# HyHuang1995/sp_orb_slam

Hardware: AMD Instinct MI355X
Metric: frames/sec SuperPoint extract (752x480, 1k kpts) (higher is better)
Workload: dtype f32

## Files before the change

sp_orb_slam_amd/csrc/conv_f32.hip:

```cpp
#include <type_traits>
#include <utility>

#include "spfe_kernels.h"
#include "../../include/spfe_exact_math.h"

namespace spfe {

typedef float f32x16 __attribute__((ext_vector_type(16)));

template <int KS, int TH>
struct Geo {
  static constexpr int HALO = KS / 2;
  static constexpr int ROWS = TH + 2 * HALO;
  static constexpr int COLS = 32 + 2 * HALO;
  static constexpr int ROWP = (KS == 3) ? 36 : 32;
  static constexpr int PLANE_RAW = ROWS * ROWP;
  static constexpr int PLANE = PLANE_RAW + ((2 - PLANE_RAW % 8) + 8) % 8;
};

typedef int i32x4 __attribute__((ext_vector_type(4)));
#define SPFE_OOB 0x80000000u

template <int NITER, int NWITER>
struct Pipe {
  float4 va[NITER];
  float4 vw[NWITER];
  int dst[NITER];
  unsigned voff[NITER];
  unsigned woff[NWITER];
  __amdgpu_buffer_rsrc_t rin, rw;
  const float *at[8];
  const float *bBase;
  float *nA, *nW;
};

template <int NR, int NT>
struct EpiCtx {
  __amdgpu_buffer_rsrc_t rout;
  unsigned rbase[NR][NT];
  float bias[NT];
  int xlim;
  unsigned pixstep;
};

__device__ __forceinline__ float max4_finite(float a, float b, float c, float d) {
  float m;
  asm("v_max3_f32 %0, %1, %2, %3\n\tv_max_f32 %0, %0, %4" : "=&v"(m) : "v"(a), "v"(b), "v"(c), "v"(d));
  return m;
}

template <int MT, int NT, bool POOL, bool RELU, int E>
__device__ __forceinline__ void epi_store(const EpiCtx<POOL ? MT / 2 : MT, NT> &e, const f32x16 (&acc)[MT][NT]) {
  constexpr int NEPI_ = POOL ? (MT / 2) * NT * 8 : MT * NT * 16;
  if constexpr (E >= NEPI_) {
    return;
  } else if constexpr (!POOL) {
    constexpr int j = E / (MT * 16), i = (E / 16) % MT, r = E % 16;
    constexpr int xr = (r & 3) + 8 * (r >> 2);
    float v = acc[i][j][r] + e.bias[j];
    if (RELU) v = v > 0.0f ? v : 0.0f;
    const unsigned off = xr < e.xlim ? e.rbase[i][j] : SPFE_OOB;
    __builtin_amdgcn_raw_buffer_store_b32(__float_as_int(v), e.rout, off, xr * e.pixstep, 0);
  } else {
    constexpr int ip = E / (NT * 8), j = (E / 8) % NT, r = 2 * (E % 8), i0 = 2 * ip;
    constexpr int xr = (r & 3) + 8 * (r >> 2);
    const float m = max4_finite(acc[i0][j][r], acc[i0][j][r + 1], acc[i0 + 1][j][r], acc[i0 + 1][j][r + 1]);
    float v = m + e.bias[j];
    if (RELU) v = v > 0.0f ? v : 0.0f;
    const unsigned off = xr < e.xlim ? e.rbase[ip][j] : SPFE_OOB;
    __builtin_amdgcn_raw_buffer_store_b32(__float_as_int(v), e.rout, off, (xr >> 1) * e.pixstep, 0);
  }
}

constexpr int F1_PROWS = 12, F1_PCOLS = 36, F1_PATCH = F1_PROWS * F1_PCOLS;

template <int NITER>
struct Fuse1a {
  float4 w[9], bias;
  float px[9];
  float4 o;
  unsigned pb[NITER];
  const float *patch;
  float *patch_next;
  const float *wsrc;
  const float *bsrc;
  __amdgpu_buffer_rsrc_t rimg;
  unsigned poff[2];
  unsigned pidx[2];
  unsigned pval[2];
  bool fill;
};
struct NoFuse {};

constexpr int F1_SUBS = 10;
template <int NITER, int IT, int SUB, int PLANE, int NWITER>
__device__ __forceinline__ void fuse_piece(Fuse1a<NITER> &z, Pipe<NITER, NWITER> &c) {
  if constexpr (SUB == 0) {
    const unsigned b = z.pb[IT] == ~0u ? 0u : z.pb[IT];
#pragma unroll
    for (int t = 0; t < 9; ++t) z.px[t] = z.patch[b + (t / 3) * F1_PCOLS + t % 3];
  } else if constexpr (SUB <= 8) {
    constexpr int j = (SUB - 1) / 2, half = (SUB - 1) % 2;
    float acc = half == 0 ? 0.0f : (j == 0 ? z.o.x : (j == 1 ? z.o.y : (j == 2 ? z.o.z : z.o.w)));
#pragma unroll
    for (int t = half * 5; t < (half == 0 ? 5 : 9); ++t) {
      const float wt = j == 0 ? z.w[t].x : (j == 1 ? z.w[t].y : (j == 2 ? z.w[t].z : z.w[t].w));
      acc = __builtin_fmaf(z.px[t], wt, acc);
    }
    if constexpr (half == 1) {
      const float bj = j == 0 ? z.bias.x : (j == 1 ? z.bias.y : (j == 2 ? z.bias.z : z.bias.w));
      acc = acc + bj;
      acc = acc > 0.0f ? acc : 0.0f;
      if (c.voff[IT] == SPFE_OOB) acc = 0.0f;
    }
    if constexpr (j == 0) z.o.x = acc;
    else if constexpr (j == 1) z.o.y = acc;
    else if constexpr (j == 2) z.o.z = acc;
    else z.o.w = acc;
  } else {
    float *d = c.nA + c.dst[IT];
    d[0] = z.o.x;
    d[PLANE] = z.o.y;
    d[2 * PLANE] = z.o.z;
    d[3 * PLANE] = z.o.w;
  }
}

template <int STEP, int NSTEP, bool FIRST, int KC, int KS, int MT, int NT, int PLANE, int ROWP, int NITER,
          int NWITER, bool POOL, bool RELU, bool FUSE, class FZ>
__device__ __forceinline__ void k_steps(float (&a)[2][MT], float (&bb)[2][NT], f32x16 (&acc)[MT][NT],
                                        const f32x16 (&accPrev)[MT][NT], Pipe<NITER, NWITER> &c,
                                        const EpiCtx<POOL ? MT / 2 : MT, NT> &e, FZ &fz) {
  if constexpr (STEP < NSTEP) {
    constexpr int NLDA = FUSE ? 0 : NITER;
    constexpr int NLD = NLDA + NWITER;
    constexpr int L0 = 1, W0 = NSTEP - NLD - 1;
    constexpr int NEPI = POOL ? (MT / 2) * NT * 8 : MT * NT * 16;
    constexpr int EPS = (NEPI + (NSTEP - 3)) / (NSTEP - 2);
    constexpr int cur = STEP & 1, nxt = cur ^ 1;
    static_assert(L0 + NLD <= W0, "loads and LDS writes of a stage must not overlap");
    constexpr int M = MT * NT;
    if constexpr (STEP >= 1) __builtin_amdgcn_s_waitcnt(0xC07F);
#pragma unroll
    for (int m = 0; m < M; ++m) {
      if (m == 0) {
        if constexpr (STEP + 1 < NSTEP) {
          constexpr int tap = (STEP + 1) / (KC / 2), t = (STEP + 1) % (KC / 2);
          constexpr int dy = tap / KS, dx = tap % KS;
#pragma unroll
          for (int i = 0; i < MT; ++i) {
            if constexpr (KC / 2 <= 8) a[nxt][i] = c.at[t][(i + dy) * ROWP + dx];
            else a[nxt][i] = c.at[0][(2 * t) * PLANE + (i + dy) * ROWP + dx];
          }
#pragma unroll
          for (int j = 0; j < NT; ++j) bb[nxt][j] = c.bBase[j * (KS * KS * KC * 32) + (tap * KC + 2 * t) * 32];
        }
      }
      if (m == 1 % M) {
        if constexpr (STEP >= L0 && STEP - L0 < NLD) {
          constexpr int it = STEP - L0;
          if constexpr (it < NLDA) {
            const i32x4 v = __builtin_amdgcn_raw_buffer_load_b128(c.rin, c.voff[it], 0, 0);
            c.va[it] = make_float4(__int_as_float(v.x), __int_as_float(v.y), __int_as_float(v.z), __int_as_float(v.w));
          } else {
            constexpr int wi = it - NLDA;
            const i32x4 v = __builtin_amdgcn_raw_buffer_load_b128(c.rw, c.woff[wi], 0, 0);
            c.vw[wi] = make_float4(__int_as_float(v.x), __int_as_float(v.y), __int_as_float(v.z), __int_as_float(v.w));
          }
        }
      }
      if (m == 2 % M) {
        if constexpr (FIRST && STEP >= 1) {
          constexpr int e0 = (STEP - 1) * EPS;
          [&]<int... Qs>(std::integer_sequence<int, Qs...>) {
            (epi_store<MT, NT, POOL, RELU, e0 + Qs>(e, accPrev), ...);
          }(std::make_integer_sequence<int, EPS>{});
        }
      }
      if (m == 3 % M) {
        if constexpr (STEP >= W0 && STEP - W0 < NLD) {
          constexpr int it = STEP - W0;
          if constexpr (it < NLDA) {
            float *d = c.nA + c.dst[it];
            d[0] = c.va[it].x;
            d[PLANE] = c.va[it].y;
            d[2 * PLANE] = c.va[it].z;
            d[3 * PLANE] = c.va[it].w;
          } else {
            constexpr int wi = it - NLDA;
            *reinterpret_cast<float4 *>(reinterpret_cast<char *>(c.nW) + c.woff[wi]) = c.vw[wi];
          }
        }
      }
      if (m == 1 % M) {
        if constexpr (FUSE) {
          constexpr int F0 = 12;
          static_assert(L0 + NLD <= F0 && F0 + F1_SUBS * NITER <= NSTEP, "fused conv1a schedule does not fit the stage");
          if constexpr (STEP >= F0 && STEP < F0 + F1_SUBS * NITER)
            fuse_piece<NITER, (STEP - F0) / F1_SUBS, (STEP - F0) % F1_SUBS, PLANE, NWITER>(fz, c);
        }
      }
      if (m == 3 % M) {
        if constexpr (FUSE) {
          static_assert(58 < W0, "fused conv1a schedule does not fit the stage");
          if constexpr (STEP >= 2 && STEP < 11) fz.w[STEP - 2] = *reinterpret_cast<const float4 *>(fz.wsrc + (STEP - 2) * 64);
          if constexpr (STEP == 11) fz.bias = *reinterpret_cast<const float4 *>(fz.bsrc);
          if constexpr (STEP == 50) {
            if (fz.fill) {
              fz.pval[0] = __builtin_amdgcn_raw_buffer_load_b8(fz.rimg, fz.poff[0], 0, 0);
              fz.pval[1] = __builtin_amdgcn_raw_buffer_load_b8(fz.rimg, fz.poff[1], 0, 0);
            }
          }
          if constexpr (STEP == 58) {
            if (fz.fill) {
              if (fz.pidx[0] < F1_PATCH) fz.patch_next[fz.pidx[0]] = spfe_pixel_to_float((uint8_t)fz.pval[0]);
              if (fz.pidx[1] < F1_PATCH) fz.patch_next[fz.pidx[1]] = spfe_pixel_to_float((uint8_t)fz.pval[1]);
            }
          }
        }
      }
      __builtin_amdgcn_sched_barrier(0);
      {
        const int i = m / NT, j = m % NT;
        if constexpr (FIRST && STEP == 0) {
          f32x16 z;
#pragma unroll
          for (int r = 0; r < 16; ++r) z[r] = 0.0f;
          acc[i][j] = __builtin_amdgcn_mfma_f32_32x32x2f32(a[cur][i], bb[cur][j], z, 0, 0, 0);
        } else {
          acc[i][j] = __builtin_amdgcn_mfma_f32_32x32x2f32(a[cur][i], bb[cur][j], acc[i][j], 0, 0, 0);
        }
      }
      __builtin_amdgcn_sched_barrier(0);
    }
    k_steps<STEP + 1, NSTEP, FIRST, KC, KS, MT, NT, PLANE, ROWP, NITER, NWITER, POOL, RELU, FUSE, FZ>(a, bb, acc, accPrev, c, e, fz);
  }
}

template <int LAYER, int CIN, int KS, int KC, int WM, int WN, int MT, int NT, bool POOL, bool RELU>
// ... 91 lines not shown
    c.rw = __builtin_amdgcn_make_buffer_rsrc(const_cast<float *>(wb), 0, valid ? (unsigned)SLAB_BYTES : 0u, 0x00020000);
  };

  aim_tile(i_tx, i_ty);
  aim_stage(i_nb, i_b, 0, true);
  FZ fz;
  [[maybe_unused]] float *sP = smem + 2 * BUF;
  [[maybe_unused]] int pcur = 0;
  [[maybe_unused]] int php[2] = {0, 0}, pwp[2] = {0, 0};
  if constexpr (FUSE) {
    const int qq = tid % Q;
#pragma unroll
    for (int it = 0; it < NITER; ++it) {
      const int i = tid + it * 256, pix = i / Q;
      fz.pb[it] = i < NITEM ? (unsigned)((pix / G::COLS) * F1_PCOLS + pix % G::COLS) : ~0u;
    }
#pragma unroll
    for (int k = 0; k < 2; ++k) {
      const int i = tid + k * 256;
      fz.pidx[k] = i < F1_PATCH ? (unsigned)i : 0xffffu;
      php[k] = i / F1_PCOLS;
      pwp[k] = i % F1_PCOLS;
      fz.poff[k] = SPFE_OOB;
      fz.pval[k] = 0u;
    }
    fz.fill = false;
    fz.patch = sP;
    fz.patch_next = sP + F1_PATCH;
    fz.rimg = __builtin_amdgcn_make_buffer_rsrc(const_cast<uint8_t *>(p.img), 0, 0u, 0x00020000);
    fz.wsrc = p.w1a + qq * 4;
    fz.bsrc = p.b1a + qq * 4;
    {
      const uint8_t *ib = p.img + (size_t)i_b * H * W;
#pragma unroll
      for (int k = 0; k < 2; ++k) {
        const int gy = i_ty * TH - 2 + php[k], gx = i_tx * 32 - 2 + pwp[k];
        const bool in = (unsigned)gy < (unsigned)H && (unsigned)gx < (unsigned)W;
        if (fz.pidx[k] < F1_PATCH) sP[fz.pidx[k]] = in ? spfe_pixel_to_float(ib[(size_t)gy * W + gx]) : 0.0f;
      }
    }
    __syncthreads();
#pragma unroll
    for (int t = 0; t < 9; ++t) fz.w[t] = *reinterpret_cast<const float4 *>(fz.wsrc + t * 64);
    fz.bias = *reinterpret_cast<const float4 *>(fz.bsrc);
    c.nA = smem;
    [&]<int... I>(std::integer_sequence<int, I...>) {
      (fuse_piece<NITER, I / F1_SUBS, I % F1_SUBS, PLANE, NWITER>(fz, c), ...);
    }(std::make_integer_sequence<int, F1_SUBS * NITER>{});
  } else {
#pragma unroll
    for (int it = 0; it < NITER; ++it) {
      const i32x4 v = __builtin_amdgcn_raw_buffer_load_b128(c.rin, c.voff[it], 0, 0);
      c.va[it] = make_float4(__int_as_float(v.x), __int_as_float(v.y), __int_as_float(v.z), __int_as_float(v.w));
    }
  }
#pragma unroll
  for (int it = 0; it < NWITER; ++it) {
    const i32x4 v = __builtin_amdgcn_raw_buffer_load_b128(c.rw, c.woff[it], 0, 0);
    c.vw[it] = make_float4(__int_as_float(v.x), __int_as_float(v.y), __int_as_float(v.z), __int_as_float(v.w));
  }
  if constexpr (!FUSE) {
#pragma unroll
    for (int it = 0; it < NITER; ++it) {
      float *d = smem + c.dst[it];
      d[0] = c.va[it].x;
      d[PLANE] = c.va[it].y;
      d[2 * PLANE] = c.va[it].z;
      d[3 * PLANE] = c.va[it].w;
    }
  }
#pragma unroll
  for (int it = 0; it < NWITER; ++it)
    *reinterpret_cast<float4 *>(reinterpret_cast<char *>(smem + KC * PLANE) + c.woff[it]) = c.vw[it];
  __syncthreads();

  f32x16 accA[MT][NT], accB[MT][NT];
#pragma unroll
  for (int i = 0; i < MT; ++i)
#pragma unroll
    for (int j = 0; j < NT; ++j)
#pragma unroll
      for (int r = 0; r < 16; ++r) { accA[i][j][r] = 0.0f; accB[i][j][r] = 0.0f; }

  constexpr int NR = POOL ? MT / 2 : MT;
  using Epi = EpiCtx<NR, NT>;
  Epi epi;
  epi.rout = __builtin_amdgcn_make_buffer_rsrc(p.out, 0, 0u, 0x00020000);
#pragma unroll
  for (int j = 0; j < NT; ++j) {
    epi.bias[j] = 0.0f;
#pragma unroll
    for (int q = 0; q < NR; ++q) epi.rbase[q][j] = SPFE_OOB;
  }
  epi.xlim = 0; epi.pixstep = out_pix_bytes;
  bool more = true;

  auto aim_epi = [&](Epi &e, int nb, int tx, int ty, int b) {
    float *obase = p.out + (size_t)b * Ho * Wo * p.out_stride + p.out_choff;
    e.rout = __builtin_amdgcn_make_buffer_rsrc(obase, 0, frame_out_bytes, 0x00020000);
    const int y0 = ty * TH + wm * MT, x0 = tx * 32 + 4 * hi;
    e.xlim = W - x0;
    e.pixstep = out_pix_bytes;
    const int ylim = H - y0;
    const unsigned rowstep = (unsigned)Wo * out_pix_bytes;
#pragma unroll
    for (int j = 0; j < NT; ++j) {
      const int co = nb * 64 + (wn * NT + j) * 32 + l31;
      const unsigned pix = POOL ? (unsigned)((y0 >> 1) * Wo + (x0 >> 1)) : (unsigned)(y0 * W + x0);
      const unsigned obase = pix * out_pix_bytes + (unsigned)co * 4u;
#pragma unroll
      for (int q = 0; q < NR; ++q)
        e.rbase[q][j] = (co < p.cout_real && (POOL ? 2 * q : q) < ylim) ? obase + q * rowstep : SPFE_OOB;
      e.bias[j] = p.bias[co];
    }
  };

  Epi epi_next;
  auto run_tile = [&](f32x16(&acc)[MT][NT], const f32x16(&accPrev)[MT][NT]) {
    int n_nb = i_nb + d_nb, n_tx = i_tx + d_tx, n_ty = i_ty + d_ty, n_b = i_b + d_b;
    if (n_nb >= p.nblk) { n_nb -= p.nblk; ++n_tx; }
    if (n_tx >= p.tiles_x) { n_tx -= p.tiles_x; ++n_ty; }
    if (n_ty >= p.tiles_y) { n_ty -= p.tiles_y; ++n_b; }
    const bool have_next_item = w + gper < hi_w;
    aim_epi(epi_next, i_nb, i_tx, i_ty, i_b);
    auto stage = [&]<bool FIRST>(std::bool_constant<FIRST>, const int chunk) {
      const bool last = chunk == NCHUNK - 1;
      if (!last) {
        aim_stage(i_nb, i_b, chunk + 1, true);
      } else {
        aim_tile(n_tx, n_ty);
        aim_stage(n_nb, n_b, 0, have_next_item);
      }
      if constexpr (FUSE) {
        const int produced = last ? 0 : chunk + 1;
        const int qq = tid % Q;
        fz.wsrc = p.w1a + produced * KC + qq * 4;
        fz.bsrc = p.b1a + produced * KC + qq * 4;
        fz.patch = sP + (last ? pcur ^ 1 : pcur) * F1_PATCH;
        fz.patch_next = sP + (pcur ^ 1) * F1_PATCH;
        fz.fill = chunk == NCHUNK - 2 && have_next_item;
        if (fz.fill) {
          fz.rimg = __builtin_amdgcn_make_buffer_rsrc(const_cast<uint8_t *>(p.img) + (size_t)n_b * H * W, 0,
                                                      (unsigned)(H * W), 0x00020000);
#pragma unroll
          for (int k = 0; k < 2; ++k) {
            const int gy = n_ty * TH - 2 + php[k], gx = n_tx * 32 - 2 + pwp[k];
            fz.poff[k] = ((unsigned)gy < (unsigned)H && (unsigned)gx < (unsigned)W) ? (unsigned)(gy * W + gx) : SPFE_OOB;
          }
        }
      }
      const int buf = chunk & 1;
      float *cA = smem + buf * BUF;
      c.nA = smem + (buf ^ 1) * BUF;
      c.nW = c.nA + KC * PLANE;
#pragma unroll
      for (int t = 0; t < (KC / 2 <= 8 ? KC / 2 : 1); ++t)
        c.at[t] = cA + (2 * t + hi) * PLANE + (wm * MT) * ROWP + l31;
      c.bBase = cA + KC * PLANE + (wn * NT) * (TAPS * KC * 32) + hi * 32 + l31;
      float a[2][MT], bb[2][NT];
#pragma unroll
      for (int i = 0; i < MT; ++i) a[0][i] = c.at[0][i * ROWP];
#pragma unroll
      for (int j = 0; j < NT; ++j) bb[0][j] = c.bBase[j * (TAPS * KC * 32)];
      k_steps<0, NSTEP, FIRST, KC, KS, MT, NT, PLANE, ROWP, NITER, NWITER, POOL, RELU, FUSE, FZ>(a, bb, acc, accPrev, c, epi, fz);
      __syncthreads();
    };
    static_assert(NCHUNK >= 2 && NCHUNK % 2 == 0, "the stage that carries the epilogue is not the tile's last; buf = chunk & 1");
    stage(std::true_type{}, 0);
#pragma unroll 1
    for (int chunk = 1; chunk < NCHUNK; ++chunk) stage(std::false_type{}, chunk);
    epi = epi_next;
    if constexpr (FUSE) pcur ^= 1;
    more = have_next_item;
    w += gper;
    i_nb = n_nb; i_tx = n_tx; i_ty = n_ty; i_b = n_b;
  };

  bool lastA = true;
  while (true) {
    run_tile(accA, accB);
    lastA = true;
    if (!more) break;
    run_tile(accB, accA);
    lastA = false;
    if (!more) break;
  }
  {
    constexpr int NEPI = POOL ? (MT / 2) * NT * 8 : MT * NT * 16;
    auto flush = [&](const f32x16(&acc)[MT][NT]) {
      [&]<int... E>(std::integer_sequence<int, E...>) {
        (epi_store<MT, NT, POOL, RELU, E>(epi, acc), ...);
      }(std::make_integer_sequence<int, NEPI>{});
    };
    if (lastA) flush(accA); else flush(accB);
  }
}

template <int LAYER, int CIN, int KS, int KC, int WM, int WN, int MT, int NT, bool POOL, bool RELU>
static hipError_t launch_one(const ConvParams &p, hipStream_t s) {
  constexpr int TH = WM * MT;
  using G = Geo<KS, TH>;
  constexpr size_t lds = (2 * (size_t)(KC * G::PLANE + KS * KS * KC * 64) + (LAYER == 2 ? 2 * F1_PATCH : 0)) * sizeof(float);
  static_assert(lds <= 160 * 1024, "double buffer must fit the 160 KB LDS");
  auto k = conv_f32_kernel<LAYER, CIN, KS, KC, WM, WN, MT, NT, POOL, RELU>;
  static LdsLimitOnce lds_once;
  if (hipError_t e = raise_lds_limit(lds_once, reinterpret_cast<const void *>(k), (int)lds); e != hipSuccess) return e;
  const int total = p.nblk * p.tiles_x * p.tiles_y * p.B;
  int grid = p.num_cus > 0 ? p.num_cus : 256;
  grid &= ~7;
  if (grid < 8) grid = 8;
  (void)total;
  hipLaunchKernelGGL(k, dim3(grid), dim3(64 * WM * WN), lds, s, p);
  return hipGetLastError();
}

int conv_kc(int ksize) { return ksize == 3 ? 16 : 64; }
int conv_tile_rows(int tile_mode) { return tile_mode == 1 ? 4 : (tile_mode == 2 || tile_mode == 4 ? 16 : (tile_mode == 3 ? 2 : 8)); }

hipError_t launch_conv_f32(const ConvParams &p, int cin, int ksize, bool pool, bool relu,
                           int tile_mode, int layer_tag, hipStream_t s) {
  const bool small_tile = tile_mode == 1;
  if (tile_mode == 3 && ksize == 3 && relu && !pool) {
    if (cin == 64) return launch_one<0, 64, 3, 16, 2, 2, 1, 1, false, true>(p, s);
    if (cin == 128) return launch_one<0, 128, 3, 16, 2, 2, 1, 1, false, true>(p, s);
    return hipErrorInvalidValue;
  }
  if (tile_mode == 4 && ksize == 3 && relu && pool && cin == 64 && layer_tag == 1)
    return launch_one<1, 64, 3, 16, 4, 1, 4, 2, true, true>(p, s);
  if (tile_mode == 2 && ksize == 3 && relu) {
    if (layer_tag == 1 && cin == 64 && pool) return launch_one<1, 64, 3, 16, 8, 1, 2, 2, true, true>(p, s);
    if (cin == 64 && pool) return launch_one<0, 64, 3, 16, 8, 1, 2, 2, true, true>(p, s);
    if (cin == 64 && !pool) return launch_one<0, 64, 3, 16, 8, 1, 2, 2, false, true>(p, s);
    if (cin == 128 && pool) return launch_one<0, 128, 3, 16, 8, 1, 2, 2, true, true>(p, s);
    if (cin == 128 && !pool) return launch_one<0, 128, 3, 16, 8, 1, 2, 2, false, true>(p, s);
    return hipErrorInvalidValue;
  }
  if (layer_tag == 1 && cin == 64 && ksize == 3 && pool && relu && !small_tile)
    return launch_one<1, 64, 3, 16, 4, 1, 2, 2, true, true>(p, s);
  if (layer_tag == 2 && cin == 64 && ksize == 3 && pool && relu && !small_tile && p.img && p.w1a && p.b1a)
    return launch_one<2, 64, 3, 16, 4, 1, 2, 2, true, true>(p, s);
#define SPFE_CONV(CIN_, KS_, KC_, WM_, WN_, MT_, NT_, POOL_, RELU_)                       \
  if (cin == CIN_ && ksize == KS_ && pool == POOL_ && relu == RELU_ &&                    \
      small_tile == (WM_ * MT_ == 4))                                                     \
    return launch_one<0, CIN_, KS_, KC_, WM_, WN_, MT_, NT_, POOL_, RELU_>(p, s);
  SPFE_CONV(64, 3, 16, 4, 1, 2, 2, true, true)
  SPFE_CONV(64, 3, 16, 4, 1, 2, 2, false, true)
  SPFE_CONV(128, 3, 16, 4, 1, 2, 2, true, true)
  SPFE_CONV(128, 3, 16, 4, 1, 2, 2, false, true)
// ... 104 lines not shown
```

sp_orb_slam_amd/csrc/spfe_host.h:

```cpp
#pragma once
#include <hip/hip_runtime.h>
#include <dlfcn.h>

#include <algorithm>
#include <chrono>
#include <functional>
#include <cfloat>
#include <cstdarg>
#include <cstdio>
#include <cstdlib>
#include <cstring>
#include <string>
#include <vector>

#include "../../include/spfe.h"
#include "../../include/spfe_exact_math.h"
#include "spfe_kernels.h"
#include "conv_plan.h"

extern "C" {
typedef struct ncclComm *ncclComm_t;
#define NCCL_UNIQUE_ID_BYTES 128
typedef struct { char internal[NCCL_UNIQUE_ID_BYTES]; } ncclUniqueId;
typedef enum { ncclSuccess = 0 } ncclResult_t;
typedef enum { ncclInt8 = 0, ncclUint8 = 1 } ncclDataType_t;
typedef ncclResult_t (*pfn_ncclGetUniqueId)(ncclUniqueId *);
typedef ncclResult_t (*pfn_ncclCommInitRank)(ncclComm_t *, int, ncclUniqueId, int);
typedef ncclResult_t (*pfn_ncclCommDestroy)(ncclComm_t);
typedef ncclResult_t (*pfn_ncclCommCount)(const ncclComm_t, int *);
typedef ncclResult_t (*pfn_ncclAllGather)(const void *, void *, size_t, ncclDataType_t, ncclComm_t, hipStream_t);
typedef const char *(*pfn_ncclGetErrorString)(ncclResult_t);
}


namespace spfe_host {

using spfe_plan::CallMode;
extern thread_local std::string g_err;
int fail(int code, const char *fmt, ...);

#define HIP_TRY(expr)                                                                   \
  do {                                                                                  \
    hipError_t e_ = (expr);                                                             \
    if (e_ != hipSuccess)                                                               \
      return ::spfe_host::fail(SPFE_EHIP, "%s failed: %s (%s:%d)", #expr, hipGetErrorString(e_), __FILE__, \
                  __LINE__);                                                            \
  } while (0)

constexpr int NSTAGE = 15;
extern const char *const kStageNames[NSTAGE];

struct ConvLayer : spfe_plan::LayerShape {
  int cout_real;
  float *d_w = nullptr, *d_b = nullptr;
  const float *in = nullptr;
  int in_stride = 0, in_choff = 0;
  float *out = nullptr;
  int out_stride = 0, out_choff = 0;
};

struct DevBuf {
  uint8_t *p = nullptr;
  size_t bytes = 0;
  template <class T>
  T *as() const { return reinterpret_cast<T *>(p); }
};

}
using spfe_host::ConvLayer;
using spfe_host::NSTAGE;

struct spfe_handle_s {
  spfe_config cfg{};
  int H = 0, W = 0, hc = 0, wc = 0, C = 0, kmax = 0, B = 0;
  hipStream_t stream = nullptr;
  hipStream_t side = nullptr;
  static constexpr int NTICKET = 4;
  hipEvent_t ev_post[NTICKET] = {}, ev_cov[NTICKET] = {};
  hipEvent_t ev_db = nullptr;
  hipEvent_t ev_desc = nullptr;
  hipStream_t conv2 = nullptr;
  std::vector<hipStream_t> conv2_pool;
  struct Conv2Choice { hipStream_t for_stream, conv2; bool ok; };
  std::vector<Conv2Choice> conv2_known;
  bool conv2_ok = false;
  long long *probe_stamp = nullptr;
  bool split_last = false;
  int split_probe = -3;
  hipEvent_t ev_fork = nullptr, ev_join = nullptr;
  bool join_pending = false;
  bool defer_join = true;
  int split_mode = -1;
  bool inline_chain = true, tail_per_half = true, sel_ext_event = true, zero_in_tail = true;
  spfe_handle twin = nullptr;
  bool is_twin = false;
  bool twin_failed = false;
  int two_chains_env = -1;
  std::vector<float> blob;
  long last_seq = 0;
  long g_ticket = 0;
  struct TicketRef { spfe_handle who; long local; } tmap[8] = {};
  int replay_waves = 0;
  int sparse_db_env = -1, sparse_da_env = -1, pbtail_env = 1, fuse1a_env = -1, pipe_copy_kernel = -1, cov_ecap_env = -1;
  bool desc_recorded = false;
  long ticket = 0;
  bool cov_inflight = false;
  std::vector<void *> dev_allocs;
  std::vector<void *> host_allocs;
  uint8_t *d_img = nullptr;
  float *d_w1a = nullptr, *d_b1a = nullptr;
  unsigned short *d_w1a_tab = nullptr;
  float *act[8] = {};
  float *d_head = nullptr, *d_semi = nullptr, *d_coarse = nullptr;
  unsigned short *d_hd = nullptr;
  unsigned char *d_wdb = nullptr, *d_wpb = nullptr;
  float *d_wdb32 = nullptr, *d_wpb32 = nullptr;
  bool f32_heads = false;
  bool pbtail = true;
  float *d_wpb_dust = nullptr;
  bool sparse_db = true;
  bool sparse_db_sync_only = false;
  bool sparse_last = false;
  bool sparse_da = false;
  int sparse_da_mode = 1;
  bool sparse_da_call = false;
  int *d_db_list = nullptr, *d_db_total = nullptr;
  int db_cap = 0;
  int db_tiles_per_wg = 4;
  hipEvent_t ev_sel = nullptr;
  hipEvent_t ev_dbs[2] = {};
  bool dbs_recorded[2] = {};
  float *act7_alt = nullptr;
  float *d_wda32 = nullptr;
  const float *feat_cur = nullptr;
  float *d_heat_log[2] = {}, *d_heat = nullptr, *d_heat_inv = nullptr;
  float *d_minmax[2] = {}, *d_cell_score[2] = {}, *d_heat_consts = nullptr;
  uint8_t *d_cell_k[2] = {}, *d_cell_mask = nullptr;
  const uint8_t *rec_of[NTICKET] = {};
  int *d_kp_cell = nullptr;
  int *d_sel_slot = nullptr;
  uint16_t *d_sel_list = nullptr;
  bool select_huge = false;
  int select_huge_env = 0;
  uint8_t *d_sel_state = nullptr;
  int *d_sel_list32 = nullptr;
  uint8_t *d_records = nullptr;
  spfe::CovScratch cov{};
  int cov_gen_code = 0;
  int cov_gen_start = 32766;
  int cov_frames_clean = 0;
  int cov_captured_min = 0;
  ConvLayer layers[10];
  spfe_plan::Switches plan_sw{};
  spfe::RecordLayout rl{};
  uint8_t *h_img = nullptr, *h_records = nullptr;
  float *h_heat = nullptr, *h_heat_inv = nullptr;
  float *own_heat = nullptr, *own_heat_inv = nullptr;
  float *usr_heat = nullptr, *usr_heat_inv = nullptr;
  int last_n = 0;
  int host_sync_n = 0;
  hipStream_t s_heat = nullptr;
  hipEvent_t ev_heat = nullptr, ev_heat_copied1 = nullptr, ev_heat_copied = nullptr;
  bool early_heat_copy = true;
  int open_n = 0;
  bool host_sync_call = false;
  bool heat_early = false;
  bool desc_early = false;
  int num_cus = 256;
  spfe_staging st{};
  bool st_set = false;
  float *d_map_x = nullptr, *d_map_y = nullptr;
  uint8_t *d_raw = nullptr, *h_raw = nullptr;
  std::vector<spfe_host::DevBuf *> grown;
  spfe_host::DevBuf stage;
  uint8_t *stage_host = nullptr;
  size_t stage_host_bytes = 0;
// ... 227 lines not shown
```

sp_orb_slam_amd/csrc/spfe_pack.hip:

```cpp
#include "spfe_host.h"

namespace spfe_host {

void make_layout(int kmax, int C, bool desc_bf16, spfe::RecordLayout *r) {
  size_t o = 0;
  r->kmax = kmax;
  r->desc_bf16 = desc_bf16 ? 1 : 0;
  r->off_hdr = o; o += 16;
  r->off_xy = o; o = align_up(o + (size_t)kmax * 2 * 4, 16);
  r->off_resp = o; o = align_up(o + (size_t)kmax * 4, 16);
  r->off_cov = o; o = align_up(o + (size_t)kmax * 2 * 4, 16);
  r->off_cinv = o; o = align_up(o + (size_t)kmax * 2 * 4, 16);
  r->off_desc = o; o = align_up(o + (size_t)kmax * SPFE_DESC_DIM * (desc_bf16 ? 2 : 4), 16);
  r->off_occ = o; o = align_up(o + (size_t)C * 2, 16);
  r->off_dd = o; o = align_up(o + (size_t)C * 4, 16);
  r->off_sd = o; o = align_up(o + (size_t)C * 4, 16);
  r->bytes = align_up(o, 256);
}

size_t blob_weight_offset(int l) {
  size_t off = 0;
  for (int i = 0; i < l; ++i) {
    const spfe_layer_t &L = SPFE_LAYERS[i];
    off += (size_t)L.cout * L.cin * L.ksize * L.ksize + L.cout;
// ... 112 lines not shown
    cout += L.cout;
  }
  if (cout % 128) return fail(SPFE_EINVAL, "internal: %d output channels are not whole 128-channel groups", cout);
  std::vector<unsigned short> wb((size_t)cout * 128 * 9);
  size_t o = 0;
  for (int i = 0; i < nl; ++i) {
    const spfe_layer_t &L = SPFE_LAYERS[lids[i]];
    const float *W = blob + blob_weight_offset(lids[i]);
    for (size_t k = 0; k < (size_t)L.cout * 128 * 9; ++k) wb[o++] = host_bf16_rne(W[k]);
  }
  std::vector<unsigned char> w((size_t)(cout / 128) * spfe::conv_bf16_rw_weight_bytes());
  spfe::conv_bf16_rw_pack_weights(wb.data(), cout, w.data());
  int rc;
  if ((rc = dev_alloc(h, out, w.size()))) return rc;
  HIP_TRY(hipMemcpy(*out, w.data(), w.size(), hipMemcpyHostToDevice));
  return SPFE_OK;
}

int load_blob(const spfe_config *cfg, std::vector<float> *blob) {
  blob->resize(SPFE_NUM_PARAMS);
  if (cfg->weights) {
    memcpy(blob->data(), cfg->weights, (size_t)SPFE_NUM_PARAMS * 4);
    return SPFE_OK;
  }
  if (!cfg->weights_path) return fail(SPFE_EWEIGHTS, "no weights: both weights and weights_path are NULL");
  FILE *f = fopen(cfg->weights_path, "rb");
  if (!f) return fail(SPFE_EWEIGHTS, "cannot open weight file %s", cfg->weights_path);
  unsigned char head[16];
  uint32_t ver = 0;
  uint64_t n = 0;
  bool ok = fread(head, 1, 16, f) == 16 && memcmp(head, "SPFW", 4) == 0;
  if (ok) {
    memcpy(&ver, head + 4, 4);
    memcpy(&n, head + 8, 8);
    ok = ver == 1 && n == SPFE_NUM_PARAMS && fread(blob->data(), 4, n, f) == n;
  }
  fclose(f);
  if (!ok) return fail(SPFE_EWEIGHTS, "%s is not a valid SPFW v1 file with %d params", cfg->weights_path, SPFE_NUM_PARAMS);
  return SPFE_OK;
}


static int env_int(const char *name, int dflt) {
  const char *e = getenv(name);
  return e && *e ? (int)strtol(e, nullptr, 0) : dflt;
}
static int env_field(const char *name, int k, int dflt) {
  const char *e = getenv(name);
  if (!e) return dflt;
  for (int i = 0; i < k; ++i) {
    e = strchr(e, ',');
    if (!e) return dflt;
    ++e;
  }
  return (*e && *e != ',') ? (int)strtol(e, nullptr, 0) : dflt;
}
static void read_switches(spfe_handle h) {
  const int st = env_int("SPFE_STAGE_TIMING", 0);
  h->timing = st != 0;
  h->timing_all = st != 2;
  h->split_mode = env_int("SPFE_SPLIT", -1);
  h->inline_chain = env_int("SPFE_INLINE_CHAIN", 1) != 0;
  h->defer_join = env_int("SPFE_DEFER_JOIN", 1) != 0;
  h->tail_per_half = env_int("SPFE_TAIL_PER_HALF", 1) != 0;
  h->two_chains_env = env_int("SPFE_TWO_CHAINS", -1);
  h->sel_ext_event = env_int("SPFE_SEL_EXT_EVENT", 1) != 0;
  h->replay_waves = env_int("SPFE_REPLAY_WAVES", 0);
  h->zero_in_tail = env_int("SPFE_ZERO_IN_TAIL", 1) != 0;
  h->sparse_db_env = env_int("SPFE_SPARSE_DB", -1);
  h->sparse_da_env = env_int("SPFE_SPARSE_DA", -1);
  h->pbtail_env = env_int("SPFE_PBTAIL", 1);
  h->f32_heads = env_int("SPFE_F32_HEADS", 0) != 0;
  h->fuse1a_env = env_int("SPFE_FUSE_CONV1A", -1);
  h->early_heat_copy = env_int("SPFE_EARLY_HEAT_COPY", 1) != 0;
  h->pipe_copy_kernel = env_int("SPFE_PIPE_COPY_KERNEL", -1);
  h->tile16x4 = env_int("SPFE_TILE16X4", 1);
  {
    const int m = env_int("SPFE_TILE2_MASK", -1);
    h->tile2_auto = m < 0;
    h->tile2_mask = m > 0 ? (unsigned)m : 0u;
  }
  h->select_huge_env = env_int("SPFE_SELECT_HUGE", 0);
  h->pool_split = env_int("SPFE_POOL_SPLIT", -1);
  h->ws_mask = (unsigned)env_field("SPFE_BF16_WS", 0, 15) & 0xfu;
  if (getenv("SPFE_BF16_WS") && strchr(getenv("SPFE_BF16_WS"), ','))
    h->ws_min_items = h->ws_min_items_sync = env_field("SPFE_BF16_WS", 1, h->ws_min_items);
  h->bf16_dyn = env_int("SPFE_BF16_DYN_QUEUE", 1) != 0;
  h->tile_rows_big = env_field("SPFE_BF16_TILE_ROWS", 0, 12);
  h->tile16_min_items = env_field("SPFE_BF16_TILE_ROWS", 1, 3);
  h->bf16_rw = env_field("SPFE_BF16_RW", 0, 1) != 0;
  h->rw_min4 = env_field("SPFE_BF16_RW", 1, 3);
  h->rw_min2 = env_field("SPFE_BF16_RW", 2, 2);
  h->rw_rows3 = env_field("SPFE_BF16_RW", 3, 1);
  h->cov.qcap = std::max(16, env_field("SPFE_COV_CAPS", 0, 1024));
  h->cov.ovf_slots = std::max(0, env_field("SPFE_COV_CAPS", 1, 16));
  h->cov.ovf_cap = std::max(h->cov.qcap, env_field("SPFE_COV_CAPS", 2, 16384));
  h->cov.fb_cap = std::max(1024, env_field("SPFE_COV_CAPS", 3, 1 << 22));
  h->cov_gen_start = std::min(32766, std::max(2, env_field("SPFE_COV_CAPS", 5, 32766)));
  h->cov_ecap_env = env_field("SPFE_COV_CAPS", 4, -1);
}

static void copy_switches(spfe_handle h, const spfe_handle_s *o) {
  h->timing = o->timing; h->timing_all = o->timing_all; h->split_mode = o->split_mode; h->inline_chain = o->inline_chain;
  h->defer_join = o->defer_join; h->tail_per_half = o->tail_per_half; h->two_chains_env = o->two_chains_env;
  h->sel_ext_event = o->sel_ext_event; h->replay_waves = o->replay_waves; h->zero_in_tail = o->zero_in_tail;
  h->sparse_db_env = o->sparse_db_env; h->sparse_da_env = o->sparse_da_env; h->pbtail_env = o->pbtail_env;
  h->f32_heads = o->f32_heads; h->fuse1a_env = o->fuse1a_env; h->pipe_copy_kernel = o->pipe_copy_kernel;
  h->early_heat_copy = o->early_heat_copy;
  h->tile16x4 = o->tile16x4; h->tile2_auto = o->tile2_auto; h->tile2_mask = o->tile2_mask;
  h->select_huge_env = o->select_huge_env; h->pool_split = o->pool_split;
  h->ws_mask = o->ws_mask; h->ws_min_items = o->ws_min_items; h->ws_min_items_sync = o->ws_min_items_sync;
  h->bf16_dyn = o->bf16_dyn; h->tile_rows_big = o->tile_rows_big; h->tile16_min_items = o->tile16_min_items;
  h->bf16_rw = o->bf16_rw; h->rw_min4 = o->rw_min4; h->rw_min2 = o->rw_min2; h->rw_rows3 = o->rw_rows3;
  h->cov.qcap = o->cov.qcap; h->cov.ovf_slots = o->cov.ovf_slots; h->cov.ovf_cap = o->cov.ovf_cap; h->cov.fb_cap = o->cov.fb_cap;
  h->cov_gen_start = o->cov_gen_start; h->cov_ecap_env = o->cov_ecap_env;
}

int build(spfe_handle h, const spfe_config *cfg, spfe_handle sibling) {
  h->cfg = *cfg;
  h->cfg.weights = nullptr;
  h->cfg.weights_path = nullptr;
  if (sibling) copy_switches(h, sibling);
  else read_switches(h);
  h->H = cfg->height; h->W = cfg->width;
  h->hc = h->H / 8; h->wc = h->W / 8; h->C = h->hc * h->wc;
  h->kmax = cfg->num_features + 1;
  h->B = cfg->max_batch;
  h->bf16 = cfg->precision == SPFE_PRECISION_BF16;
  const int H = h->H, W = h->W, B = h->B, C = h->C;
  HIP_TRY(hipSetDevice(cfg->device));
  {
    hipDeviceProp_t prop;
    HIP_TRY(hipGetDeviceProperties(&prop, cfg->device));
    h->num_cus = prop.multiProcessorCount;
  }
  HIP_TRY(hipStreamCreateWithFlags(&h->stream, hipStreamNonBlocking));
  HIP_TRY(hipStreamCreateWithFlags(&h->side, hipStreamNonBlocking));
  for (int i = 0; i < spfe_handle_s::NTICKET; ++i) {
    HIP_TRY(hipEventCreateWithFlags(&h->ev_post[i], hipEventDisableTiming));
    HIP_TRY(hipEventCreateWithFlags(&h->ev_cov[i], hipEventDisableTiming));
  }
  HIP_TRY(hipEventCreateWithFlags(&h->ev_desc, hipEventDisableTiming));
  HIP_TRY(hipEventCreateWithFlags(&h->ev_fork, hipEventDisableTiming));
  HIP_TRY(hipEventCreateWithFlags(&h->ev_join, hipEventDisableTiming));
  HIP_TRY(hipEventCreateWithFlags(&h->ev_db, hipEventDisableTiming));
  HIP_TRY(hipEventCreateWithFlags(&h->ev_sel, hipEventDisableTiming));
  for (int i = 0; i < 2; ++i) HIP_TRY(hipEventCreateWithFlags(&h->ev_dbs[i], hipEventDisableTiming));
  h->sparse_db = true;
  h->sparse_db_sync_only = h->bf16 && h->C < 10000;
  h->db_tiles_per_wg = h->bf16 ? 4 : 1;
  if (h->sparse_db_env >= 0) { h->sparse_db = h->sparse_db_env != 0; h->sparse_db_sync_only = h->sparse_db_env == 2; }
  if ((size_t)cfg->max_batch * h->C * (h->bf16 ? 1024 : 2048) >= ((size_t)1 << 31))
    return fail(SPFE_EINVAL, "internal: max_batch %d x %d cells passed spfe_create's whole-call limit", cfg->max_batch, h->C);
  h->fuse1a = !h->bf16 && h->fuse1a_env > 0;
  h->fuse1a_bf16 = h->bf16 && h->fuse1a_env != 0;
  if (h->timing) {
    h->evpool.resize((size_t)spfe_handle_s::EVSETS * (NSTAGE + 1), nullptr);
    for (auto &e : h->evpool) HIP_TRY(hipEventCreate(&e));
  }

  int rc;
  if (!sibling) {
    if ((rc = load_blob(cfg, &h->blob))) return rc;
  } else if (sibling->blob.size() != (size_t)SPFE_NUM_PARAMS) return fail(SPFE_EWEIGHTS, "internal: the sibling's weight blob is gone");
  const std::vector<float> &blob = sibling ? sibling->blob : h->blob;

  {
    const float *Wt = blob.data() + blob_weight_offset(0);
    std::vector<float> w(9 * 64), bv(64);
    for (int co = 0; co < 64; ++co) {
      for (int t = 0; t < 9; ++t) w[t * 64 + co] = Wt[co * 9 + t];
      bv[co] = Wt[64 * 9 + co];
    }
    if ((rc = dev_alloc(h, &h->d_w1a, w.size()))) return rc;
    if ((rc = dev_alloc(h, &h->d_b1a, bv.size()))) return rc;
    HIP_TRY(hipMemcpy(h->d_w1a, w.data(), w.size() * 4, hipMemcpyHostToDevice));
    HIP_TRY(hipMemcpy(h->d_b1a, bv.data(), bv.size() * 4, hipMemcpyHostToDevice));
    if (h->bf16) {
      std::vector<unsigned short> tab(2 * 64 * 8, 0);
      for (int j = 0; j < 2; ++j)
        for (int ln = 0; ln < 64; ++ln)
          for (int e = 0; e < 8; ++e) {
            const int t = 8 * (ln >> 5) + e, m = ln & 31, co = 32 * j + ((m & ~12) | ((m & 4) << 1) | ((m & 8) >> 1));
            if (t < 9) tab[(j * 64 + ln) * 8 + e] = host_bf16_rne(Wt[co * 9 + t] * (1.0f / 255.0f));
          }
      if ((rc = dev_alloc(h, &h->d_w1a_tab, tab.size()))) return rc;
      HIP_TRY(hipMemcpy(h->d_w1a_tab, tab.data(), tab.size() * 2, hipMemcpyHostToDevice));
    }
  }

  const int lh[8] = {H, H / 2, H / 2, H / 4, H / 4, H / 8, H / 8, H / 8};
  const int lw[8] = {W, W / 2, W / 2, W / 4, W / 4, W / 8, W / 8, W / 8};
  const int lc[8] = {64, 64, 64, 64, 128, 128, 128, 128};
// ... 180 lines not shown
```

sp_orb_slam_amd/csrc/spfe_schedule.hip:

```cpp
#include "spfe_host.h"

namespace spfe_host {

hipError_t wait_if_pending(hipStream_t s, hipEvent_t ev) {
  hipStreamCaptureStatus cs = hipStreamCaptureStatusNone;
  if (hipStreamIsCapturing(s, &cs) == hipSuccess && cs == hipStreamCaptureStatusNone) {
    const hipError_t q = hipEventQuery(ev);
    if (q == hipSuccess) return hipSuccess;
    if (q != hipErrorNotReady) (void)hipGetLastError();
  }
  return hipStreamWaitEvent(s, ev, 0);
}

#define STAGE_MARK(i) \
  do { if (h->timing && (h->timing_all || (i) == 1 || (i) == 2)) HIP_TRY(hipEventRecord(h->ev[i], s)); } while (0)

}
namespace spfe {
__global__ void copy_records_kernel(uint4 *dst, const uint4 *src, size_t n16) {
  for (size_t i = (size_t)blockIdx.x * blockDim.x + threadIdx.x; i < n16; i += (size_t)gridDim.x * blockDim.x) dst[i] = src[i];
  __threadfence_system();
}

__global__ void queue_probe_spin_kernel(long long ticks, long long *stamp) {
// ... 48 lines not shown
  for (int k = 0; k < 4; ++k) {
    if ((int)h->conv2_pool.size() <= k) {
      hipStream_t c = nullptr;
      HIP_TRY(hipStreamCreateWithFlags(&c, hipStreamNonBlocking));
      h->conv2_pool.push_back(c);
    }
    hipStream_t c = h->conv2_pool[k];
    const int q1 = streams_share_a_queue(c, s, h->probe_stamp);
    const int q2 = q1 == 0 ? streams_share_a_queue(c, h->side, h->probe_stamp) : q1;
    if (q1 < 0 || q2 < 0) h->split_probe = -1;
    if (q1 == 0 && q2 == 0) {
      h->conv2 = c;
      h->conv2_ok = true;
      h->split_probe = 1;
      break;
    }
  }
  return SPFE_OK;
}

int settle_join(spfe_handle h, hipStream_t s) {
  if (h->join_pending) {
    HIP_TRY(wait_if_pending(s, h->ev_join));
    h->join_pending = false;
  }
  return SPFE_OK;
}

using namespace spfe_plan;

CallMode call_mode(const spfe_handle_s *h, int n) {
  return CallMode{(h->cfg.flags & SPFE_FLAG_ASYNC_COV) || h->pipe_mode, h->timing && h->timing_all,
                  h->num_cus > 0 ? h->num_cus : 256, h->bf16, n, false};
}

int enqueue(spfe_handle h, const uint8_t *d_images, int n, uint8_t *d_records, hipStream_t s) {
  const int H = h->H, W = h->W;
  if (h->open_n) return fail(SPFE_EINVAL, "a call begun by spfe_extract_begin is open: spfe_extract_finish first");
  if (h->timing) h->ev = h->evpool.data() + (size_t)(h->calls % spfe_handle_s::EVSETS) * (NSTAGE + 1);
  h->calls++;
  h->host_sync_n = 0;
  STAGE_MARK(0);
  if (h->bf16) { const int rcj = settle_join(h, s); if (rcj) return rcj; }
  if (h->d_tile_ctr && !h->tile_ctr_clean) {
    hipLaunchKernelGGL(spfe::zero_tile_counters_kernel, dim3(1), dim3(256), 0, s, h->d_tile_ctr, 8 * 64);
    HIP_TRY(hipGetLastError());
  }
  h->tile_ctr_clean = false;
  CallMode m = call_mode(h, n);
  const bool sparse = h->sparse_db && h->d_db_list && !(h->sparse_db_sync_only && m.pipelined);
  m.sparse_da = sparse && h->sparse_da && (h->sparse_da_mode >= 2 || !m.pipelined);
  h->sparse_da_call = m.sparse_da;
  h->act0_missing = plan_conv(h->layers[0], 0, n, m, h->plan_sw).first == 2;
  const bool early_waits = h->split_last && h->pbtail && n >= 2 && m.pipelined && !m.stage_events;
  if (early_waits) { const int rcw = tail_waits(h, d_records, s); if (rcw) return rcw; }
  if (!h->act0_missing && h->bf16) HIP_TRY(spfe::launch_conv1a_bf16(d_images, h->d_w1a_tab, h->d_b1a, h->act[0], n, H, W, s));
  else if (!h->act0_missing) HIP_TRY(spfe::launch_conv1a(d_images, h->d_w1a, h->d_b1a, h->act[0], n, H, W, s));
  { const int rcj = settle_join(h, s); if (rcj) return rcj; }
  STAGE_MARK(1);
  const int par_db = (int)(h->ticket & 1);
  h->feat_cur = m.sparse_da && par_db ? h->act7_alt : h->act[7];
  bool tail_per_half = false;
  auto run_layer = [&](int i, int f0, int n, hipStream_t s) -> int {
    const ConvLayer &L = h->layers[i];
    if (i == 9 && h->desc_recorded) HIP_TRY(wait_if_pending(s, h->ev_desc));
    if (!m.sparse_da && i == 7 && h->dbs_recorded[par_db ^ 1]) HIP_TRY(wait_if_pending(s, h->ev_dbs[par_db ^ 1]));
    if (m.sparse_da && i == 6 && h->dbs_recorded[par_db]) HIP_TRY(wait_if_pending(s, h->ev_dbs[par_db]));
    const ConvPlan c = plan_conv(L, i, n, m, h->plan_sw);
    const int part = f0 > 0 ? 1 : 0;
    spfe::ConvParams p{};
    p.in = L.in; p.in_stride = L.in_stride; p.in_choff = L.in_choff; p.bias = L.d_b;
    p.wpack = c.family == Family::Bf16Ws ? reinterpret_cast<const float *>(h->d_wws[i])
              : c.family == Family::Bf16Rw ? reinterpret_cast<const float *>(h->d_wrw[i - 4]) : L.d_w;
    p.out = L.out; p.out_stride = L.out_stride; p.out_choff = L.out_choff; p.cout_real = L.cout_real;
    if (m.sparse_da && i == 6) p.out = const_cast<float *>(h->feat_cur);
    if (m.sparse_da && i == 7) p.in = h->feat_cur;
    p.B = n; p.H = L.H; p.W = L.W;
    const size_t esz = h->bf16 ? 2 : 4, out_px = L.pool ? (size_t)(L.H / 2) * (L.W / 2) : (size_t)L.H * L.W;
    p.in = reinterpret_cast<const float *>(reinterpret_cast<const char *>(p.in) + (size_t)f0 * L.H * L.W * L.in_stride * esz);
    p.out = reinterpret_cast<float *>(reinterpret_cast<char *>(p.out) + f0 * out_px * L.out_stride * esz);
    if (h->bf16 && i == 7) { p.out = reinterpret_cast<float *>(h->d_hd + (size_t)f0 * h->C * 512); p.out_stride = 512; p.out_choff = 0; }
    if (c.first == 2) { p.img = d_images; p.w1a = h->bf16 ? reinterpret_cast<const float *>(h->d_w1a_tab) : h->d_w1a; p.b1a = h->d_b1a; }
    p.tiles_x = c.tiles_x; p.tiles_y = c.tiles_y; p.nblk = c.nblk; p.num_cus = h->num_cus;
    if (c.queue) p.tile_ctr = h->d_tile_ctr + 64 * i + 32 * part;
    if (i == 0 && !h->bf16) { h->conv1b_tile_rows = c.rows; h->conv1b_split_rows = (int)c.split16_rows; }
    switch (c.family) {
      case Family::InTail:
        if (tail_per_half) {
          const spfe::FrameBufs fb = frame_bufs(h, d_records, sparse);
          if (h->bf16) {
            HIP_TRY(spfe::launch_pbtail_bf16(h->d_hd, h->d_wpb, h->layers[8].d_b, h->d_semi, fb, h->rl, n, H, W, s, f0,
                                             h->d_tile_ctr ? h->d_tile_ctr + 32 * part : nullptr, h->d_tile_ctr ? 8 * 32 : 0, 64,
                                             h->pbtail_env > 1 ? h->pbtail_env : 0));
            if (h->d_tile_ctr) h->tile_ctr_clean = true;
          } else HIP_TRY(spfe::launch_pbtail_f32(h->d_head, h->d_wpb32, h->d_wpb_dust, h->layers[8].d_b, h->d_semi, fb, h->rl, n, H, W, s, f0));
        }
        break;
      case Family::Head:
        if (h->bf16)
          HIP_TRY(spfe::launch_head1x1_bf16(h->d_hd + (size_t)f0 * h->C * 512, i == 8 ? h->d_wpb : h->d_wdb, L.d_b,
                                            L.out + (size_t)f0 * h->C * L.out_stride, n * h->C, L.cout_real, s));
        else HIP_TRY(spfe::launch_head1x1_f32(h->d_head, i == 8 ? h->d_wpb32 : h->d_wdb32, L.d_b, L.out, n * h->C, L.cout_real, s));
        break;
      case Family::Bf16Ws: HIP_TRY(spfe::launch_conv_bf16_ws(p, L.pool, c.first, s)); break;
      case Family::Bf16Rw: HIP_TRY(spfe::launch_conv_bf16_rw(p, L.pool, c.tile, s)); break;
      case Family::Bf16Streamed: HIP_TRY(spfe::launch_conv_bf16(p, L.cin, L.pool, false, s, c.tile)); break;
      case Family::F32PoolSplit: {
        spfe::ConvParams q = p;
        q.out = h->d_unpooled; q.out_stride = L.out_stride; q.out_choff = 0;
        HIP_TRY(spfe::launch_conv_f32(q, L.cin, L.ks, false, true, c.tile, 0, s));
        HIP_TRY(spfe::launch_pool2x2_f32(h->d_unpooled, p.out, n, L.H, L.W, L.out_stride, s));
        break;
      }
      case Family::F32Split16: {
        spfe::ConvParams p16 = p;
        p16.tiles_y = c.tiles_y16; p16.item_lo = 0; p16.item_hi = c.hi16;
        HIP_TRY(spfe::launch_conv_f32(p16, L.cin, L.ks, L.pool, L.relu, 4, 1, s));
        const bool kernel_bracket = h->timing && !h->timing_all;
        if (kernel_bracket) HIP_TRY(hipEventRecord(h->ev[2], s));
        p.item_lo = c.lo8; p.item_hi = c.hi8;
        HIP_TRY(spfe::launch_conv_f32(p, L.cin, L.ks, L.pool, L.relu, 0, 1, s));
        if (kernel_bracket) return SPFE_OK;
        break;
      }
      case Family::F32: HIP_TRY(spfe::launch_conv_f32(p, L.cin, L.ks, L.pool, L.relu, c.tile, c.first, s)); break;
    }
    STAGE_MARK(2 + i);
    return SPFE_OK;
  };
  const bool defer_db = !sparse && !m.stage_events && !m.pipelined;
  const int nlayers = sparse ? 9 : 10;
  bool split = (h->split_mode >= 0 ? h->split_mode >= 1 : (!h->bf16 || h->C < 10000)) && !(!h->bf16 && h->f32_heads) && n >= 2 && !m.stage_events && !defer_db;
  if (split) { const int rcp = pick_conv2(h, s); if (rcp) return rcp; }
  h->split_last = split = split && h->conv2_ok;
  if (split) {
    tail_per_half = h->pbtail && h->tail_per_half;
    if (tail_per_half && !early_waits) { const int rcw = tail_waits(h, d_records, s); if (rcw) return rcw; }
    int rc = run_layer(0, 0, n, s);
    if (rc) return rc;
    HIP_TRY(hipEventRecord(h->ev_fork, s));
    HIP_TRY(hipStreamWaitEvent(h->conv2, h->ev_fork, 0));
    for (int i = 1; i < nlayers; ++i)
      for (int r = 0; r < 2; ++r) {
        const int f0 = r * (n / 2), nfr = r ? n - n / 2 : n / 2;
        if ((rc = run_layer(i, f0, nfr, r ? h->conv2 : s))) return rc;
      }
    HIP_TRY(hipEventRecord(h->ev_join, h->conv2));
    if (tail_per_half && h->defer_join && m.pipelined) h->join_pending = true;
    else HIP_TRY(hipStreamWaitEvent(s, h->ev_join, 0));
    return enqueue_post(h, m, d_records, s, nullptr, sparse, h->pbtail, tail_per_half);
  }
  for (int i = 0; i < (defer_db ? 9 : nlayers); ++i) { const int rc = run_layer(i, 0, n, s); if (rc) return rc; }
  if (sparse) STAGE_MARK(2 + 9);
  if (!defer_db) return enqueue_post(h, m, d_records, s, nullptr, sparse, h->pbtail);
  const std::function<int()> conv_db = [&]() -> int { return run_layer(9, 0, n, s); };
  return enqueue_post(h, m, d_records, s, &conv_db, false, h->pbtail);
}

int launch_db_gathered(spfe_handle h, int n, hipStream_t s) {
  const ConvLayer &L = h->layers[9];
  const int max_total = n * h->db_cap;
  if (h->bf16 && h->sparse_da_call)
    HIP_TRY(spfe::launch_da_gather_bf16(h->feat_cur, h->d_wrw[3], h->layers[7].d_b, h->d_hd, h->d_db_list, h->d_db_total, max_total, n, h->hc, h->wc, h->num_cus, s));
  if (!h->bf16 && h->sparse_da_call)
    HIP_TRY(spfe::launch_da_gather_f32(h->feat_cur, h->d_wda32, h->layers[7].d_b + 256, h->d_head, h->d_db_list, h->d_db_total, max_total, n, h->hc, h->wc, h->num_cus, s));
  if (h->bf16) HIP_TRY(spfe::launch_head1x1_bf16_gather(h->d_hd, h->d_wdb, L.d_b, h->d_coarse, n * h->C, h->d_db_list, h->d_db_total, max_total, h->db_tiles_per_wg, s));
// ... 215 lines not shown
```

Before: 2173.

## Carry next stage's first LDS operands across the stage barrier in f32 conv

For the non-fused f32 conv path, the last k-step of each stage now issues the barrier itself and then prefetches the first A/B operands of the next buffer by flipping the LDS base pointers. This removes the trailing barrier and the cold operand reload at the start of every stage. For NT==1 it also loads the B operand for two steps at once. The change adds an env knob (SPFE_GRID_CUS) that caps the CU count used for persistent-grid sizing, and it forces the stage lambdas to inline. The cost is more live registers and a slightly shorter window for LDS writes.

```diff
diff --git a/sp_orb_slam_amd/csrc/conv_f32.hip b/sp_orb_slam_amd/csrc/conv_f32.hip
--- a/sp_orb_slam_amd/csrc/conv_f32.hip
+++ b/sp_orb_slam_amd/csrc/conv_f32.hip
@@ -19,6 +19,7 @@
 };
 
 typedef int i32x4 __attribute__((ext_vector_type(4)));
+constexpr int pipe_bases(int KC, int MT) { return KC / 2 <= 8 && MT > 1 ? KC / 2 : 1; }
 #define SPFE_OOB 0x80000000u
 
 template <int NITER, int NWITER>
@@ -32,6 +33,8 @@
   const float *at[8];
   const float *bBase;
   float *nA, *nW;
+  int flip;
+  float b1;
 };
 
 template <int NR, int NT>
@@ -134,13 +137,16 @@
   if constexpr (STEP < NSTEP) {
     constexpr int NLDA = FUSE ? 0 : NITER;
     constexpr int NLD = NLDA + NWITER;
-    constexpr int L0 = 1, W0 = NSTEP - NLD - 1;
+    constexpr bool CARRY = !FUSE;
+    constexpr int L0 = 1, W0 = NSTEP - NLD - (CARRY ? 2 : 1);
+    static_assert(NSTEP % 2 == 0, "step 0 of every stage takes its operands from a[0] / bb[0]");
     constexpr int NEPI = POOL ? (MT / 2) * NT * 8 : MT * NT * 16;
     constexpr int EPS = (NEPI + (NSTEP - 3)) / (NSTEP - 2);
     constexpr int cur = STEP & 1, nxt = cur ^ 1;
     static_assert(L0 + NLD <= W0, "loads and LDS writes of a stage must not overlap");
     constexpr int M = MT * NT;
-    if constexpr (STEP >= 1) __builtin_amdgcn_s_waitcnt(0xC07F);
+    if constexpr (STEP >= 1 || CARRY) __builtin_amdgcn_s_waitcnt(0xC07F);
+    if constexpr (CARRY && STEP == NSTEP - 1) __syncthreads();
 #pragma unroll
     for (int m = 0; m < M; ++m) {
       if (m == 0) {
@@ -149,12 +155,36 @@
           constexpr int dy = tap / KS, dx = tap % KS;
 #pragma unroll
           for (int i = 0; i < MT; ++i) {
-            if constexpr (KC / 2 <= 8) a[nxt][i] = c.at[t][(i + dy) * ROWP + dx];
+            if constexpr (pipe_bases(KC, MT) > 1) a[nxt][i] = c.at[t][(i + dy) * ROWP + dx];
             else a[nxt][i] = c.at[0][(2 * t) * PLANE + (i + dy) * ROWP + dx];
           }
-#pragma unroll
-          for (int j = 0; j < NT; ++j) bb[nxt][j] = c.bBase[j * (KS * KS * KC * 32) + (tap * KC + 2 * t) * 32];
+          if constexpr (CARRY && NT == 1) {
+            constexpr int off = (tap * KC + 2 * t) * 32;
+            if constexpr (STEP % 2 == 0) {
+              bb[nxt][0] = c.b1;
+            } else {
+              static_assert((KC / 2) % 2 == 0 && t % 2 == 0, "an even step and the next one share a tap");
+              bb[nxt][0] = c.bBase[off];
+              c.b1 = c.bBase[off + 2 * 32];
+            }
+          } else {
+#pragma unroll
+            for (int j = 0; j < NT; ++j) bb[nxt][j] = c.bBase[j * (KS * KS * KC * 32) + (tap * KC + 2 * t) * 32];
+          }
+        } else if constexpr (CARRY) {
+          c.at[0] += c.flip;
+          c.bBase += c.flip;
+#pragma unroll
+          for (int i = 0; i < MT; ++i) a[nxt][i] = c.at[0][i * ROWP];
+#pragma unroll
+          for (int j = 0; j < NT; ++j) bb[nxt][j] = c.bBase[j * (KS * KS * KC * 32)];
+          if constexpr (NT == 1) c.b1 = c.bBase[2 * 32];
         }
+      }
+      if constexpr (CARRY && STEP == NSTEP - 1) {
+#pragma unroll
+        for (int t = 1; t < pipe_bases(KC, MT); ++t)
+          if (t % M == m) c.at[t] += c.flip;
       }
       if (m == 1 % M) {
         if constexpr (STEP >= L0 && STEP - L0 < NLD) {
@@ -412,6 +442,21 @@
 #pragma unroll
       for (int r = 0; r < 16; ++r) { accA[i][j][r] = 0.0f; accB[i][j][r] = 0.0f; }
 
+  float a[2][MT], bb[2][NT];
+  auto aim_lds = [&](int buf) {
+    const float *cA = smem + buf * BUF;
+#pragma unroll
+    for (int t = 0; t < pipe_bases(KC, MT); ++t)
+      c.at[t] = cA + (2 * t + hi) * PLANE + (wm * MT) * ROWP + l31;
+    c.bBase = cA + KC * PLANE + (wn * NT) * (TAPS * KC * 32) + hi * 32 + l31;
+#pragma unroll
+    for (int i = 0; i < MT; ++i) a[0][i] = c.at[0][i * ROWP];
+#pragma unroll
+    for (int j = 0; j < NT; ++j) bb[0][j] = c.bBase[j * (TAPS * KC * 32)];
+    if constexpr (!FUSE && NT == 1) c.b1 = c.bBase[2 * 32];
+  };
+  if constexpr (!FUSE) aim_lds(0);
+
   constexpr int NR = POOL ? MT / 2 : MT;
   using Epi = EpiCtx<NR, NT>;
   Epi epi;
@@ -446,14 +491,14 @@
   };
 
   Epi epi_next;
-  auto run_tile = [&](f32x16(&acc)[MT][NT], const f32x16(&accPrev)[MT][NT]) {
+  auto run_tile = [&](f32x16(&acc)[MT][NT], const f32x16(&accPrev)[MT][NT]) __attribute__((always_inline)) {
     int n_nb = i_nb + d_nb, n_tx = i_tx + d_tx, n_ty = i_ty + d_ty, n_b = i_b + d_b;
     if (n_nb >= p.nblk) { n_nb -= p.nblk; ++n_tx; }
     if (n_tx >= p.tiles_x) { n_tx -= p.tiles_x; ++n_ty; }
     if (n_ty >= p.tiles_y) { n_ty -= p.tiles_y; ++n_b; }
     const bool have_next_item = w + gper < hi_w;
     aim_epi(epi_next, i_nb, i_tx, i_ty, i_b);
-    auto stage = [&]<bool FIRST>(std::bool_constant<FIRST>, const int chunk) {
+    auto stage = [&]<bool FIRST>(std::bool_constant<FIRST>, const int chunk) __attribute__((always_inline)) {
       const bool last = chunk == NCHUNK - 1;
       if (!last) {
         aim_stage(i_nb, i_b, chunk + 1, true);
@@ -480,20 +525,12 @@
         }
       }
       const int buf = chunk & 1;
-      float *cA = smem + buf * BUF;
       c.nA = smem + (buf ^ 1) * BUF;
       c.nW = c.nA + KC * PLANE;
-#pragma unroll
-      for (int t = 0; t < (KC / 2 <= 8 ? KC / 2 : 1); ++t)
-        c.at[t] = cA + (2 * t + hi) * PLANE + (wm * MT) * ROWP + l31;
-      c.bBase = cA + KC * PLANE + (wn * NT) * (TAPS * KC * 32) + hi * 32 + l31;
-      float a[2][MT], bb[2][NT];
-#pragma unroll
-      for (int i = 0; i < MT; ++i) a[0][i] = c.at[0][i * ROWP];
-#pragma unroll
-      for (int j = 0; j < NT; ++j) bb[0][j] = c.bBase[j * (TAPS * KC * 32)];
+      c.flip = buf ? -BUF : BUF;
+      if constexpr (FUSE) aim_lds(buf);
       k_steps<0, NSTEP, FIRST, KC, KS, MT, NT, PLANE, ROWP, NITER, NWITER, POOL, RELU, FUSE, FZ>(a, bb, acc, accPrev, c, epi, fz);
-      __syncthreads();
+      if constexpr (FUSE) __syncthreads();
     };
     static_assert(NCHUNK >= 2 && NCHUNK % 2 == 0, "the stage that carries the epilogue is not the tile's last; buf = chunk & 1");
     stage(std::true_type{}, 0);
diff --git a/sp_orb_slam_amd/csrc/spfe_host.h b/sp_orb_slam_amd/csrc/spfe_host.h
--- a/sp_orb_slam_amd/csrc/spfe_host.h
+++ b/sp_orb_slam_amd/csrc/spfe_host.h
@@ -92,6 +92,7 @@
   bool defer_join = true;
   int split_mode = -1;
   bool inline_chain = true, tail_per_half = true, sel_ext_event = true, zero_in_tail = true;
+  int grid_cus = 0;
   spfe_handle twin = nullptr;
   bool is_twin = false;
   bool twin_failed = false;
diff --git a/sp_orb_slam_amd/csrc/spfe_pack.hip b/sp_orb_slam_amd/csrc/spfe_pack.hip
--- a/sp_orb_slam_amd/csrc/spfe_pack.hip
+++ b/sp_orb_slam_amd/csrc/spfe_pack.hip
@@ -218,6 +218,7 @@
   }
   h->select_huge_env = env_int("SPFE_SELECT_HUGE", 0);
   h->pool_split = env_int("SPFE_POOL_SPLIT", -1);
+  h->grid_cus = std::max(0, env_int("SPFE_GRID_CUS", 0)) & ~7;
   h->ws_mask = (unsigned)env_field("SPFE_BF16_WS", 0, 15) & 0xfu;
   if (getenv("SPFE_BF16_WS") && strchr(getenv("SPFE_BF16_WS"), ','))
     h->ws_min_items = h->ws_min_items_sync = env_field("SPFE_BF16_WS", 1, h->ws_min_items);
@@ -244,7 +245,7 @@
   h->f32_heads = o->f32_heads; h->fuse1a_env = o->fuse1a_env; h->pipe_copy_kernel = o->pipe_copy_kernel;
   h->early_heat_copy = o->early_heat_copy;
   h->tile16x4 = o->tile16x4; h->tile2_auto = o->tile2_auto; h->tile2_mask = o->tile2_mask;
-  h->select_huge_env = o->select_huge_env; h->pool_split = o->pool_split;
+  h->select_huge_env = o->select_huge_env; h->pool_split = o->pool_split; h->grid_cus = o->grid_cus;
   h->ws_mask = o->ws_mask; h->ws_min_items = o->ws_min_items; h->ws_min_items_sync = o->ws_min_items_sync;
   h->bf16_dyn = o->bf16_dyn; h->tile_rows_big = o->tile_rows_big; h->tile16_min_items = o->tile16_min_items;
   h->bf16_rw = o->bf16_rw; h->rw_min4 = o->rw_min4; h->rw_min2 = o->rw_min2; h->rw_rows3 = o->rw_rows3;
diff --git a/sp_orb_slam_amd/csrc/spfe_schedule.hip b/sp_orb_slam_amd/csrc/spfe_schedule.hip
--- a/sp_orb_slam_amd/csrc/spfe_schedule.hip
+++ b/sp_orb_slam_amd/csrc/spfe_schedule.hip
@@ -154,6 +154,7 @@
     if (h->bf16 && i == 7) { p.out = reinterpret_cast<float *>(h->d_hd + (size_t)f0 * h->C * 512); p.out_stride = 512; p.out_choff = 0; }
     if (c.first == 2) { p.img = d_images; p.w1a = h->bf16 ? reinterpret_cast<const float *>(h->d_w1a_tab) : h->d_w1a; p.b1a = h->d_b1a; }
     p.tiles_x = c.tiles_x; p.tiles_y = c.tiles_y; p.nblk = c.nblk; p.num_cus = h->num_cus;
+    if (!h->bf16 && h->grid_cus > 0) p.num_cus = std::min(h->grid_cus, h->num_cus);
     if (c.queue) p.tile_ctr = h->d_tile_ctr + 64 * i + 32 * part;
     if (i == 0 && !h->bf16) { h->conv1b_tile_rows = c.rows; h->conv1b_split_rows = (int)c.split16_rows; }
     switch (c.family) {
```

Result: no change. 2193, median of 6 (+0.9%).
